# ilia-glushchenko/SimplePathTracer

Hardware: AMD Instinct MI355X
Metric: Msamples/s (pixels×spp/s), RTIOW random-sphere scene, 1/2/4/8 MI355X (higher is better)
Workload: dtype f32

## Files before the change

### simplepathtracer_amd/csrc/spt_batch.cpp

```cpp
#include "spt_host.h"

namespace spt_api {

int grow_host_rects(spt_ctx *ctx, BatchSet *bs, size_t n)
{
    if (bs->h_rects_cap >= n) return SPT_OK;
    if (int rc = svc_end(ctx)) return rc;
    const size_t cap = std::max<size_t>({n, 2 * bs->h_rects_cap, 64});
    if (bs->h_rects) HIP_TRY(ctx, hipHostFree(bs->h_rects));
    bs->h_rects = nullptr;
    bs->h_rects_cap = 0;
    HIP_TRY(ctx, hipHostMalloc((void **)&bs->h_rects, cap * sizeof(spt::BatchRect)));
    bs->h_rects_cap = cap;
    return SPT_OK;
}

void destroy_batch_set(BatchSet *b)
{
    if (b->d_rects) (void)hipFree(b->d_rects);
    if (b->h_rects) (void)hipHostFree(b->h_rects);
    if (b->d_stage) (void)hipFree(b->d_stage);
    if (b->stream) (void)hipStreamDestroy(b->stream);
}

// ... 154 lines not shown
    fa.spp_total = spp;
    fa.s_done = spp;
    fa.first = fa.last = 1;
    fa.mode = mode;
    fa.rects = bs->d_rects;
    fa.n_rects = (uint32_t)n;
    fa.inline_rects = inl ? 1u : 0u;
    if (inl)
        for (size_t i = 0; i < n; ++i) fa.rects_inline[i] = bs->h_rects[i];
    fa.head_reset = !use_svc ? w->d_head : nullptr;
    fa.head_queues = ra.n_queues;
    fa.prio = use_svc ? 0 : 1;
    EventPair ef = get_pair(ctx);
    HIP_TRY(ctx, hipEventRecord(ef.a, s));
    HIP_TRY(ctx, spt::launch_fold(fa, s));
    w->head_clean = !use_svc;
    HIP_TRY(ctx, hipEventRecord(ef.b, s));
    ctx->pending_fold.push_back(ef);

    for (size_t i = 0; i < n; ++i) {
        const BatchReq *r = batch[i];
        const spt::BatchRect &b = bs->h_rects[i];
        if (r->rgba)
            HIP_TRY(ctx, hipMemcpyAsync(r->rgba, bs->d_stage + b.pix_off, (size_t)b.npix * sizeof(float4),
                                        hipMemcpyDeviceToHost, s));
        if (r->g_data && !spec_d8 && b.rgb8 == ctx->d_frame8) {
            const size_t pitch = (size_t)W * 3, off = band_offset(W, H, r->yE, r->xB);
            HIP_TRY(ctx, hipMemcpy2DAsync(r->g_data + off, pitch, ctx->d_frame8 + off, pitch, (size_t)b.w * 3, b.rows,
                                          hipMemcpyDeviceToHost, s));
        }
    }
// ... 83 lines not shown
```

### simplepathtracer_amd/csrc/spt_ctx.cpp

```cpp
#include "spt_host.h"

namespace spt_api {

thread_local std::string g_thread_error;
thread_local const spt_ctx *t_in_callback = nullptr;

int fail(spt_ctx *ctx, int code, const char *fmt, ...)
{
    char buf[512];
    va_list ap;
    va_start(ap, fmt);
    vsnprintf(buf, sizeof buf, fmt, ap);
    va_end(ap);
    if (ctx) ctx->err = buf;
    g_thread_error = buf;
    return code;
}

void host_trace(const char *what, const void *arg)
{
    static const bool on = env_var("SPT_HOST_TRACE") && std::atoi(env_var("SPT_HOST_TRACE")) != 0;
    if (!on) return;
    static const auto t0 = std::chrono::steady_clock::now();
    const double ms = std::chrono::duration<double, std::milli>(std::chrono::steady_clock::now() - t0).count();
// ... 129 lines not shown
            uint32_t j = 0;
            while (x != 0.f && j < spt::kCodeSat) {
                x = x * 0.5f;
                ++j;
            }
            jz = std::max(jz, j);
        }
    return jz;
}

uint32_t code_jmax(const spt_ctx *ctx)
{
    return std::min(ctx->bounces > 0 ? ctx->bounces - 1u : 0u, ctx->code_jz);
}

spt::DeviceScene device_scene(const spt_ctx *ctx)
{
    return spt::DeviceScene{ctx->d_shade, ctx->d_mat, ctx->n, ctx->code_stride, code_jmax(ctx), ctx->accel};
}

int check_ready(spt_ctx *ctx)
{
    if (!ctx->scene_set) return fail(ctx, SPT_ERR_STATE, "scene not set (spt_set_scene)");
    if (!ctx->cam_set) return fail(ctx, SPT_ERR_STATE, "camera not set (spt_set_camera)");
    if (!ctx->params_set) return fail(ctx, SPT_ERR_STATE, "params not set (spt_set_params)");
    if (!spt::code_layout_fits(ctx->code_stride, code_jmax(ctx)))
        return fail(ctx, SPT_ERR_ARG,
                    "%u sphere slots at depth %u exceed the sample code space ((jmax + 1) * slots + 1 <= %u, jmax = %u)",
                    ctx->code_stride, ctx->bounces, spt::kCodeMax, code_jmax(ctx));
    return SPT_OK;
// ... 151 lines not shown
            shade[j] = ctx->h_shade[t.orig[j]];
            mat[j] = ctx->h_mat[t.orig[j]];
        }
    HIP_TRY(ctx, hipDeviceSynchronize());
    int rc = upload(ctx, &ctx->d_slots, &ctx->slots_cap, t.slots);
    if (!rc) rc = upload(ctx, &ctx->d_shade, &ctx->shade_cap, shade);
    if (!rc) rc = upload(ctx, &ctx->d_mat, &ctx->mat_cap, mat);
    if (!rc) rc = upload(ctx, &ctx->d_orig, &ctx->orig_cap, t.orig);
    if (!rc) rc = upload(ctx, &ctx->d_nodes, &ctx->nodes_cap, t.nodes);
    if (!rc) rc = upload(ctx, &ctx->d_kpre, &ctx->kpre_cap, t.kpre);
    if (rc) return rc;
    ctx->accel = spt::AccelView{ctx->d_slots, ctx->d_orig, ctx->d_nodes, t.always_groups, t.n_nodes,
                                t.n_nodes > t.leaves ? 1u : 0u, t.leaf_slots, ctx->d_kpre, t.pre_cm};
    ctx->code_stride = (uint32_t)std::max<size_t>(t.slots.size(), 1);
    ctx->code_jz = jz;
    ctx->tables = std::move(t);
    ctx->accel_gen++;
    ctx->accel_build_s = std::chrono::duration<double>(std::chrono::steady_clock::now() - t_start).count();
    return SPT_OK;
}

int wait_own_renders(spt_ctx *ctx)
{
    for (const EventPair &p : ctx->pending_render) HIP_TRY(ctx, hipEventSynchronize(p.b));
    return SPT_OK;
}

int rebuild_prim(spt_ctx *ctx)
{
    const bool want = ctx->prim_enabled && ctx->scene_set && ctx->cam_set && ctx->params_set &&
// ... 269 lines not shown
    if (const char *e = env_var("SPT_SVC_FULL_GRID"))
        if (std::atoi(e) != 0) {
            ctx->svc_grid = (uint32_t)(per_cu * ctx->num_cu);
            ctx->svc_full = true;
        }
    if (const char *e = env_var("SPT_BLOCKS_PER_CU")) per_cu = std::max(1, std::atoi(e));
    if (const char *e = env_var("SPT_CLAIM")) ctx->claim = (uint32_t)std::max(0, std::atoi(e));
    if (const char *e = env_var("SPT_CLUSTER_K")) ctx->cluster_k = (uint32_t)std::max(0, std::atoi(e));
    if (const char *e = env_var("SPT_TREE_B")) ctx->tree_branching = (uint32_t)std::max(0, std::atoi(e));
    if (const char *e = env_var("SPT_CLAIMS_PER_WAVE")) ctx->claims_per_wave = (uint32_t)std::max(1, std::atoi(e));
    if (const char *e = env_var("SPT_QUEUES"))
        ctx->queues = (uint32_t)std::min<int>((int)spt::kMaxQueues, std::max(1, std::atoi(e)));
    if (const char *e = env_var("SPT_WF_CAP")) ctx->wf_cap = (uint32_t)std::max(1024, std::atoi(e));
    if (const char *e = env_var("SPT_WF_QUEUE")) ctx->wf_queue = (uint32_t)std::min(8192, std::max(1, std::atoi(e) / 256)) * 256u;
    if (const char *e = env_var("SPT_HOST_GRID_DIV")) ctx->host_grid_div = (uint32_t)std::max(0, std::atoi(e));
    if (const char *e = env_var("SPT_BATCH")) ctx->batching = std::atoi(e) != 0;
    if (const char *e = env_var("SPT_READAHEAD")) ctx->readahead = std::atoi(e) != 0;
    if (const char *e = env_var("SPT_READAHEAD_PARTS"))
        ctx->spec.parts = (uint32_t)std::min(SpecFrame::kParts, std::max(1, std::atoi(e)));
    if (const char *e = env_var("SPT_BATCH_DBUF")) ctx->batch_dbuf = std::atoi(e) != 0;
    if (const char *e = env_var("SPT_BATCH_GRID_DIV")) ctx->batch_grid_div = (uint32_t)std::max(1, std::atoi(e));
    if (const char *e = env_var("SPT_BATCH_SETS"))
        ctx->batch_sets = (uint32_t)std::min<int>((int)kMaxBatchSets, std::max(1, std::atoi(e)));
    if (const char *e = env_var("SPT_HOST_SLOTS"))
        ctx->host_slots = (uint32_t)std::min<int>((int)kMaxHostSlots, std::max(1, std::atoi(e)));
    if (const char *e = env_var("SPT_SERVICE")) ctx->svc.enabled = std::atoi(e) != 0;
    if (const char *e = env_var("SPT_SVC_CLAIM")) ctx->svc.claim = (uint32_t)std::max(64, std::atoi(e) / 64 * 64);
    if (const char *e = env_var("SPT_SVC_LDS")) ctx->svc.lds = std::atoi(e) != 0;
    if (const char *e = env_var("SPT_SVC_QUEUES"))
        ctx->svc.queues = (uint32_t)std::min<int>((int)spt::kMaxQueues, std::max(1, std::atoi(e)));
// ... 315 lines not shown
```

### simplepathtracer_amd/csrc/spt_host.h

```cpp
#pragma once
#include "spt_hip.h"
#include "spt_accel.h"
#include "spt_internal.h"
#include "spt_readahead.h"

#include <hip/hip_runtime.h>

#include <algorithm>
#include <atomic>
#include <chrono>
#include <cmath>
#include <condition_variable>
#include <cstdarg>
#include <cstdint>
#include <cstdio>
#include <cstdlib>
#include <cstring>
#include <functional>
#include <mutex>
#include <string>
#include <thread>
#include <utility>
#include <vector>

// ... 166 lines not shown
    struct PrimKey {
        float view[12], eye[3];
        uint32_t W, H, prim_max;
        uint64_t accel_gen;
        bool valid;
        bool same(const PrimKey &o) const
        {
            return valid && o.valid && std::memcmp(view, o.view, sizeof view) == 0 &&
                   std::memcmp(eye, o.eye, sizeof eye) == 0 && W == o.W && H == o.H && prim_max == o.prim_max &&
                   accel_gen == o.accel_gen;
        }
    } prim_key{};
    uint64_t accel_gen = 0;
    uint32_t prim_blocks = 0, prim_entries = 0;
    uint32_t code_stride = 1, code_jz = 0;
    bool scene_set = false;
    std::vector<float> h_centers, h_radii;
    std::vector<float4> h_shade;
    std::vector<uint32_t> h_mat;
    uint32_t cluster_k = SPT_CLUSTER_AUTO;
    uint32_t tree_branching = SPT_TREE_AUTO;
    int engine = SPT_ENGINE_MEGAKERNEL;
    uint32_t wf_cap = 1u << 24;
    uint32_t wf_queue = 4096;
    spt::AccelView accel{};
    spt::Camera cam{};
    bool cam_set = false;
    uint32_t W = 0, H = 0, spp = 0, bounces = 0;
    uint64_t seed = 0;
    bool params_set = false;
// ... 92 lines not shown
int check_not_in_callback(spt_ctx *ctx);
int rebuild_prim(spt_ctx *ctx);
int wait_own_renders(spt_ctx *ctx);
int rebuild_accel(spt_ctx *ctx);
int ensure_wavefront(spt_ctx *ctx, Workspace *w, uint32_t cap, uint32_t qcap);
hipStream_t companion_for(spt_ctx *ctx, hipStream_t s);
Workspace * workspace_for(spt_ctx *ctx, hipStream_t s);
uint32_t render_grid(const spt_ctx *ctx, uint64_t items, uint32_t claim, uint32_t div, bool masked = false);
uint32_t claim_size(const spt_ctx *ctx, uint64_t items, bool masked = false);
int masked_for(spt_ctx *ctx, hipStream_t s, spt_ctx::Masked **out);
uint32_t full_grid(const spt_ctx *ctx, bool masked = false);
uint64_t fmix64(uint64_t z);
int check_ready(spt_ctx *ctx);
spt::DeviceScene device_scene(const spt_ctx *ctx);
uint32_t code_jmax(const spt_ctx *ctx);
uint32_t halvings_to_zero(const std::vector<float4> &shade);
double busy_ms(const spt_ctx *ctx);
int collect_timings(spt_ctx *ctx, bool wait = true);
EventPair get_pair(spt_ctx *ctx);
int check_on_device(spt_ctx *ctx, const void *p, const char *what);
int fail(spt_ctx *ctx, int code, const char *fmt, ...);
int svc_retire(spt_ctx *ctx, hipStream_t s, uint64_t w0, uint64_t words, uint32_t idx);
int svc_submit(spt_ctx *ctx, const spt::RenderArgs &ra, int mode, hipStream_t s, uint64_t *w0_out, uint32_t *idx_out);
int svc_submit_jobs(spt_ctx *ctx, int mode, const SvcJobSpec *jobs, size_t n, uint64_t total_slots, hipStream_t s, uint64_t *w0_out, uint32_t *idx_out);
bool svc_eligible(const spt_ctx *ctx, uint64_t words, bool keep_samples);
void host_trace(const char *what, const void *arg = nullptr);
void warm_start(spt_ctx *ctx);
hipStream_t warm_take(spt_ctx *ctx, int i);
void warm_join(spt_ctx *ctx);
uint32_t svc_session_grid(const spt_ctx *ctx);
// ... 68 lines not shown
```

### simplepathtracer_amd/csrc/spt_internal.h

```cpp
#pragma once
#include <hip/hip_runtime.h>
#include <stdint.h>

#include "spt_hip.h"

namespace spt {

struct RowMap {
    uint32_t y0, y1, strip, parts, part;
    uint32_t x0, width;
};

__host__ __device__ inline uint32_t row_of(const RowMap &m, uint32_t lr)
{
    uint32_t blk = lr / m.strip;
    return m.y0 + (blk * m.parts + m.part) * m.strip + (lr - blk * m.strip);
}

__host__ __device__ inline uint32_t rows_owned(const RowMap &m)
{
    if (m.y1 <= m.y0) return 0;
    uint32_t h = m.y1 - m.y0;
    uint32_t period = m.strip * m.parts;
    uint32_t full = h / period, rem = h % period;
// ... 25 lines not shown
        const uint32_t t = qb / th;
        if (t < ft) {
            const uint32_t e = qb - t * th;
            row = e >> 3;
            c = (t << 3) | (e & 7u);
        } else {
            const uint32_t e = qb - ft * th;
            row = e / wr;
            c = (ft << 3) + (e - row * wr);
        }
    }
    lr = (band << 3) + row;
    col = c;
}

struct FastDiv {
    uint32_t d, m, s;
};
inline FastDiv make_fastdiv(uint32_t d)
{
    FastDiv f{d, 0u, 0u};
    if (d <= 1u) return f;
    uint32_t l = 0;
    while ((1ull << l) < d) ++l;
    f.m = (uint32_t)(((1ull << (31 + l)) / d) + 1ull);
    f.s = l - 1u;
    return f;
}
__host__ __device__ inline uint32_t fast_div(uint32_t x, const FastDiv &f)
{
#ifdef __HIP_DEVICE_COMPILE__
    const uint32_t hi = __umulhi(x, f.m);
#else
    const uint32_t hi = (uint32_t)(((uint64_t)x * f.m) >> 32);
#endif
    return f.d <= 1u ? x : hi >> f.s;
}

__host__ __device__ inline uint32_t row_of_fast(const RowMap &m, uint32_t lr, const FastDiv &div_strip)
{
    const uint32_t blk = fast_div(lr, div_strip);
    return m.y0 + (blk * m.parts + m.part) * m.strip + (lr - blk * m.strip);
}

__host__ __device__ inline void ts_item(uint32_t q, uint32_t width, uint32_t rows, uint32_t S, const FastDiv &div_band,
                                        const FastDiv &div_tile, uint32_t &sl, uint32_t &lr, uint32_t &col)
{
    const uint32_t band = rows >= 8u ? fast_div(q, div_band) : 0u;
    const uint32_t h = rows - (band << 3) < 8u ? rows - (band << 3) : 8u;
    const uint32_t qb = q - band * 8u * width * S;
    const uint32_t ft = width >> 3, wr = width & 7u;
    const uint32_t ti = h * 8u * S;
    uint32_t e, wt, c0;
// ... 24 lines not shown
}

__host__ __device__ inline void ts_slot_base(uint32_t lr, uint32_t col, uint32_t width, uint32_t rows, uint32_t S,
                                             uint32_t &q0, uint32_t &step)
{
    const uint32_t band = lr >> 3;
    const uint32_t h = rows - (band << 3) < 8u ? rows - (band << 3) : 8u;
    const uint32_t ft = width >> 3, wr = width & 7u;
    const uint32_t t = col >> 3;
    const uint32_t tc = t < ft ? t : ft;
    const uint32_t wt = t < ft ? 8u : wr;
    q0 = band * 8u * width * S + tc * h * 8u * S + (lr - (band << 3)) * wt + (col - (tc << 3));
    step = h * wt;
}

constexpr uint32_t kCodeSmall = 0x33800000u;
constexpr uint32_t kCodeMax = 2u * (kCodeSmall - 1u);
constexpr uint32_t kCodeSat = 280;
__host__ __device__ inline bool code_layout_fits(uint64_t stride, uint32_t jmax)
{
    return (jmax + 1ull) * stride + 1ull <= kCodeMax;
}
__host__ __device__ inline uint32_t diffuse_code(uint32_t j, uint32_t slot, uint32_t stride)
{
    return 2u + j * stride + slot;
}
__host__ __device__ inline void diffuse_decode(uint32_t c, const FastDiv &div, uint32_t &j, uint32_t &slot)
{
    const uint32_t v = c - 2u;
    j = fast_div(v, div);
    slot = v - j * div.d;
}
__host__ __device__ inline uint32_t code_word(uint32_t c)
{
    return c < kCodeSmall ? c : 0x80000000u | (c - kCodeSmall + 1u);
}
__host__ __device__ inline uint32_t word_code(uint32_t w)
{
    const uint32_t a = w & 0x7FFFFFFFu;
    if (a == 0u || a >= kCodeSmall) return 0u;
    return (w >> 31) ? a + kCodeSmall - 1u : a;
}
constexpr uint32_t kZeroWord = 1u;

constexpr uint32_t kMaxGroup = 16;
constexpr uint32_t kClusterSlots = 8;
constexpr uint32_t kFlatLeafSlots = 4;
constexpr double kFlatScale = 1.0 - 1e-4;
constexpr double kBoxS = 1.63e-3;
constexpr float kBoxMinDir = 0x1p-20f;
constexpr uint32_t kNoSlot = 0xFFFFFFFFu;
constexpr uint32_t kMiss = 0xFFFFFFFFu;

struct AccelView {
    const float4 *slots;
    const uint32_t *orig;
    const void *nodes;
    uint32_t always_groups, n_nodes;
// ... 94 lines not shown
constexpr uint32_t kSvcHostCommitted = 0, kSvcHostClosing = 32, kSvcHostPub = 64, kSvcHostStop = 96,
                   kSvcHostWatchdog = 128, kSvcHostWords = 160;
constexpr uint32_t kSvcTraceClaims = 1u << 21;
hipError_t launch_render_svc(const RenderArgs &a, uint32_t grid, hipStream_t s);
bool svc_supported(const AccelView &ac);
bool svc_lds(const AccelView &ac);
uint32_t svc_lds_grid(bool full);
uint32_t svc_block(const AccelView &ac);

struct FoldArgs {
    const uint32_t *samples;
    uint32_t slot_words;
    const float4 *shade;
    float sky[3];
    FastDiv code_div;
    float4 *acc;
    float4 *out_rgba;
    uint8_t *out_rgb8;
    RowMap map;
    uint32_t width, height, npix, spp_batch, spp_total;
    uint32_t s_done;
    int first, last, mode;
    int preview;
    int prio;
    int alias;
    const BatchRect *rects;
    uint32_t n_rects;
    uint32_t range_alias, out_i0, alias_h, src_rows;
    uint32_t *head_reset;
    uint32_t head_queues;
// ... 40 lines not shown
```

### simplepathtracer_amd/csrc/spt_kernels.hip

```cpp
#include "spt_path.h"

#include <algorithm>
#include <mutex>

namespace spt {


#ifndef SPT_WAVES_PER_EU
#define SPT_WAVES_PER_EU 0
#endif
#ifndef SPT_NUM_SGPR
#define SPT_NUM_SGPR 96
#endif
#if SPT_WAVES_PER_EU
#define SPT_RENDER_ATTR __attribute__((amdgpu_waves_per_eu(SPT_WAVES_PER_EU, SPT_WAVES_PER_EU)))
#elif SPT_NUM_SGPR
#define SPT_CAP_WAVES (800 / (((SPT_NUM_SGPR - 2 + 15) / 16) * 16 + 16) > 8 ? 8 : 800 / (((SPT_NUM_SGPR - 2 + 15) / 16) * 16 + 16))
#define SPT_RENDER_ATTR __attribute__((amdgpu_num_sgpr(SPT_NUM_SGPR), amdgpu_waves_per_eu(SPT_CAP_WAVES)))
#else
#define SPT_RENDER_ATTR
#endif

#ifndef SPT_LDS_BLOCK
#define SPT_LDS_BLOCK 1024
// ... 160 lines not shown
        const uint32_t j = cur + lane;
        const uint32_t v = j < njobs ? __hip_atomic_load(jc + j, __ATOMIC_RELAXED, __HIP_MEMORY_SCOPE_AGENT) : 0xFFFFFFFFu;
        const unsigned long long le = __ballot(v <= nb);
        if (le != ~0ull || cur + 64u >= njobs) {
            if (le != 0ull) cur += 63u - (uint32_t)__builtin_clzll(le);
            break;
        }
        cur += 64u;
    }
    const gu32 *src = (const gu32 *)(k.svc_jobs + cur);
    const uint32_t w = lane < 24u ? __hip_atomic_load(src + lane, __ATOMIC_RELAXED, __HIP_MEMORY_SCOPE_AGENT) : 0u;
    if (lane < 24u) rec[lane] = w;
    return __builtin_amdgcn_readfirstlane(cur);
}

__device__ __forceinline__ float halve_n(float x, uint32_t j)
{
    if (j <= 126u) {
        const float r = x * __uint_as_float((127u - j) << 23);
        if (__builtin_fabsf(r) >= 0x1p-126f || x == 0.f || !__builtin_isfinite(x)) return r;
    }
    for (uint32_t i = 0; i < j; ++i) x = x * 0.5f;
    return x;
}
__device__ __forceinline__ f3 decode_sample(const FoldArgs &a, uint32_t w)
{
    const uint32_t c = word_code(w);
    if (c == 0u) {
        const float k = __uint_as_float(w);
        return mul(mk(a.sky[0] * k, a.sky[1] * k, a.sky[2] * k), 0.5f);
    }
    if (c == 1u) return mk(0.f, 0.f, 0.f);
    uint32_t j, slot;
    diffuse_decode(c, a.code_div, j, slot);
    const float4 sh = a.shade[slot];
    return mk(halve_n(sh.x * 0.5f, j), halve_n(sh.y * 0.5f, j), halve_n(sh.z * 0.5f, j));
}

template <int N>
__device__ __forceinline__ void decode_run(const FoldArgs &a, const uint32_t (&w)[N], f3 (&col)[N])
{
    uint32_t c[N], j[N];
    float4 sh[N];
#pragma unroll
    for (int i = 0; i < N; ++i) {
        c[i] = word_code(w[i]);
        uint32_t slot;
        diffuse_decode(c[i] >= 2u ? c[i] : 2u, a.code_div, j[i], slot);
        sh[i] = a.shade[slot];
    }
#pragma unroll
    for (int i = 0; i < N; ++i) {
        const float k = __uint_as_float(w[i]);
        const f3 s = mul(mk(a.sky[0] * k, a.sky[1] * k, a.sky[2] * k), 0.5f);
        const f3 d = mk(halve_n(sh[i].x * 0.5f, j[i]), halve_n(sh[i].y * 0.5f, j[i]), halve_n(sh[i].z * 0.5f, j[i]));
        col[i] = c[i] == 0u ? s : c[i] == 1u ? mk(0.f, 0.f, 0.f) : d;
    }
}

#ifndef SPT_FOLD_RUN
#define SPT_FOLD_RUN 8
#endif
constexpr int kFoldDecode = SPT_FOLD_RUN < 8 ? SPT_FOLD_RUN : 8;
static_assert(SPT_FOLD_RUN % kFoldDecode == 0, "fold runs are decoded kFoldDecode words at a time");

__device__ __forceinline__ void alias_accumulate(const FoldArgs &a, const uint32_t *samples, uint32_t p, uint32_t W,
                                                 uint32_t H, uint32_t row0, uint32_t rows, uint32_t S, float4 &acc)
{
    const uint32_t dy_lo = p >= W ? (p - W + H) / H : 0u;
    const uint32_t dy_hi = min(H - 1u, p / H);
    const uint32_t ns = dy_hi + 1u - dy_lo;
    const uint2 *s2 = (const uint2 *)samples;
    auto add = [&](uint32_t w) {
        const f3 c = decode_sample(a, w);
        acc.x = acc.x + c.x;
        acc.y = acc.y + c.y;
        acc.z = acc.z + c.z;
        acc.w = acc.w + 1.f;
    };
    constexpr uint32_t kSrc = 4;
    if (ns <= kSrc) {
        uint32_t sq[kSrc], sst[kSrc];
#pragma unroll
        for (uint32_t j = 0; j < kSrc; ++j) {
            const uint32_t dy = j < ns ? dy_lo + j : dy_lo;
            ts_slot_base(dy - row0, p - dy * H, W, rows, S, sq[j], sst[j]);
        }
        const bool rev = W < H;
        for (uint32_t k = 0; k < S; ++k) {
// ... 32 lines not shown
                    const uint32_t key = s2[q].y;
                    const uint64_t kp = ((uint64_t)key << 32) | (dy * W + dx);
                    if (key != 0u && kp > prev && kp < best) {
                        best = kp;
                        best_slot = q;
                    }
                }
                if (best == ~0ull) break;
                add(s2[best_slot].x);
                prev = best;
            }
        }
    }
}

__device__ __forceinline__ void fold_pixel(const FoldArgs &a, const uint32_t *samples, const RowMap &map,
                                           uint32_t rows, int alias, uint32_t lr, uint32_t col, float4 *out_rgba,
                                           uint8_t *out_rgb8)
{
    const uint32_t W = map.width, S = a.spp_batch;
    const uint32_t p = lr * W + col;
    float4 acc = a.first ? make_float4(0.f, 0.f, 0.f, 0.f) : a.acc[p];
    uint32_t q0, step;
    ts_slot_base(lr, col, W, rows, S, q0, step);
    if (a.mode == 0) {
        constexpr int kFoldRun = SPT_FOLD_RUN;
        uint32_t k = 0;
        for (; k + kFoldRun <= S; k += kFoldRun) {
            uint32_t w[kFoldRun];
#pragma unroll
            for (int i = 0; i < kFoldRun; ++i) w[i] = samples[q0 + (k + i) * step];
#pragma unroll
            for (int g = 0; g < kFoldRun; g += kFoldDecode) {
                uint32_t w8[kFoldDecode];
#pragma unroll
                for (int i = 0; i < kFoldDecode; ++i) w8[i] = w[g + i];
                f3 c[kFoldDecode];
                decode_run<kFoldDecode>(a, w8, c);
#pragma unroll
                for (int i = 0; i < kFoldDecode; ++i) {
                    acc.x = acc.x + c[i].x;
                    acc.y = acc.y + c[i].y;
                    acc.z = acc.z + c[i].z;
                    acc.w = acc.w + 1.f;
                }
            }
        }
        for (; k < S; ++k) {
            const f3 c = decode_sample(a, samples[q0 + k * step]);
            acc.x = acc.x + c.x;
            acc.y = acc.y + c.y;
            acc.z = acc.z + c.z;
            acc.w = acc.w + 1.f;
        }
    } else if (!alias) {
        const uint2 *s2 = (const uint2 *)samples;
        for (uint32_t k = 0; k < S; ++k) {
            const uint2 v = s2[q0 + k * step];
            if (v.y != 0u) {
                const f3 c = decode_sample(a, v.x);
                acc.x = acc.x + c.x;
                acc.y = acc.y + c.y;
                acc.z = acc.z + c.z;
                acc.w = acc.w + 1.f;
            }
        }
    } else {
        alias_accumulate(a, samples, p, W, rows, 0u, rows, S, acc);
    }
    if (!a.last) {
        a.acc[p] = acc;
        if (!a.preview) return;
    }
    const float scale = a.mode == 0 ? 1.f / (float)a.s_done : 1.f / acc.w;
    const float r = acc.x * scale, g = acc.y * scale, b = acc.z * scale;
    if (out_rgba) out_rgba[p] = make_float4(r, g, b, 0.f);
    if (out_rgb8) {
        const uint32_t x = map.x0 + col;
        const uint32_t y = row_of(map, lr);
        const size_t gi = (size_t)3 * ((size_t)(a.height - 1u - y) * a.width + x);
        out_rgb8[gi + 0] = gamma_byte(r);
        out_rgb8[gi + 1] = gamma_byte(g);
        out_rgb8[gi + 2] = gamma_byte(b);
// ... 502 lines not shown
{
    render_body<true, (int)kClusterSlots, true, kLdsBlock>(a);
}
__global__ __launch_bounds__(kLdsBlock)
    __attribute__((amdgpu_num_sgpr(SPT_LDS_NUM_SGPR), amdgpu_waves_per_eu(2 * kLdsBlock / 256))) void render_kernel_lds_batch(RenderArgs a)
{
    render_body<true, (int)kClusterSlots, true, kLdsBlock, true>(a);
}

__global__ __launch_bounds__(kLdsBlock)
    __attribute__((amdgpu_num_sgpr(SPT_LDS_NUM_SGPR), amdgpu_waves_per_eu(2 * kLdsBlock / 256))) void render_kernel_svc_lds(RenderArgs a)
{
    render_body<true, (int)kClusterSlots, true, kLdsBlock, false, false, true>(a);
}

#ifndef SPT_FOLD_PRIO
#define SPT_FOLD_PRIO 3
#endif
#ifndef SPT_FOLD_BLOCK
#define SPT_FOLD_BLOCK 256
#endif
__global__ __launch_bounds__(SPT_FOLD_BLOCK) void fold_kernel(FoldArgs a)
{
    if (a.prio) __builtin_amdgcn_s_setprio(SPT_FOLD_PRIO);
    const uint32_t i = blockIdx.x * blockDim.x + threadIdx.x;
    if (i >= a.npix) return;
    const uint32_t rows = a.npix / a.map.width;
    uint32_t lr, col;
    tile_pixel(i, a.map.width, rows, lr, col);
    fold_pixel(a, a.samples, a.map, rows, a.alias, lr, col, a.out_rgba, a.out_rgb8);
}

__global__ __launch_bounds__(256) void fold_alias_range_kernel(FoldArgs a)
{
    if (a.prio) __builtin_amdgcn_s_setprio(3);
    const uint32_t t = blockIdx.x * blockDim.x + threadIdx.x;
    if (t >= a.npix) return;
    float4 acc = a.first ? make_float4(0.f, 0.f, 0.f, 0.f) : a.acc[t];
    alias_accumulate(a, a.samples, a.out_i0 + t, a.map.width, a.alias_h, a.map.y0, a.src_rows, a.spp_batch, acc);
    if (!a.last) {
        a.acc[t] = acc;
        if (!a.preview) return;
    }
    const float scale = 1.f / acc.w;
    if (a.out_rgba) a.out_rgba[t] = make_float4(acc.x * scale, acc.y * scale, acc.z * scale, 0.f);
}

typedef __attribute__((address_space(4))) const BatchRect crect_k;
__device__ __forceinline__ uint32_t fold_rect(crect_k *rs, uint32_t n, uint32_t i)
{
    uint32_t lo = 0, hi = n;
    while (hi - lo > 1u) {
        const uint32_t mid = (lo + hi) >> 1;
        if (rs[mid].pix_off <= i) lo = mid; else hi = mid;
    }
    return lo;
}

__global__ __launch_bounds__(256) void fold_kernel_batch(FoldArgs a)
{
#ifndef SPT_FOLD_PRIO_BATCH
#define SPT_FOLD_PRIO_BATCH 1
#endif
    if (SPT_FOLD_PRIO_BATCH && a.prio) __builtin_amdgcn_s_setprio(3);
    const uint32_t i = blockIdx.x * blockDim.x + threadIdx.x;
    if (blockIdx.x == 0 && a.head_reset && threadIdx.x < a.head_queues) a.head_reset[threadIdx.x * kQueueStride] = 0u;
    if (i >= a.npix) return;
    typedef __attribute__((address_space(4))) const FoldArgs cfold_t;
    typedef __attribute__((address_space(4))) const char kchar;
    cfold_t *ka = (cfold_t *)(kchar *)__builtin_amdgcn_kernarg_segment_ptr();
    crect_k *rs = a.inline_rects ? (crect_k *)ka->rects_inline : (crect_k *)a.rects;
    crect_k &r = rs[fold_rect(rs, a.n_rects, i)];
    const RowMap map{r.y0, r.y0 + r.rows, 1u, 1u, 0u, r.x0, r.w};
    uint32_t lr, col;
    tile_pixel(i - r.pix_off, r.w, r.rows, lr, col);
    fold_pixel(a, a.samples + (size_t)a.slot_words * r.slot_off, map, r.rows, (int)r.alias, lr, col,
               a.out_rgba ? a.out_rgba + r.pix_off : nullptr, r.rgb8);
}

__global__ __launch_bounds__(256) void expand_kernel(FoldArgs a, float4 *out, uint32_t p0, uint32_t n)
{
    const uint32_t i = blockIdx.x * blockDim.x + threadIdx.x;
    if (i >= n) return;
    const uint32_t p = p0 + i;
    const uint32_t W = a.map.width, rows = a.npix / W, lr = p / W, col = p - lr * W;
    uint32_t q0, step;
    ts_slot_base(lr, col, W, rows, a.spp_batch, q0, step);
    for (uint32_t k = 0; k < a.spp_batch; ++k) {
        const uint32_t q = q0 + k * step;
        const uint32_t w = a.slot_words == 1u ? a.samples[q] : a.samples[2u * q];
        const bool counted = a.slot_words == 1u || a.samples[2u * q + 1u] != 0u;
        const f3 c = decode_sample(a, w);
        out[(size_t)i * a.spp_batch + k] = make_float4(c.x, c.y, c.z, counted ? 1.f : 0.f);
    }
}

__global__ __launch_bounds__(256) void assemble_kernel(const float4 *tiles, uint32_t max_rows, RowMap base,
                                                       uint32_t width, uint32_t height, float4 *frame, uint8_t *rgb8)
{
    const uint32_t x = blockIdx.x * blockDim.x + threadIdx.x;
    const uint32_t k = blockIdx.y;
    const uint32_t r = blockIdx.z;
    if (x >= base.width) return;
    RowMap m = base;
    m.part = r;
    if (k >= rows_owned(m)) return;
    const uint32_t y = row_of(m, k);
// ... 129 lines not shown
        return hipGetLastError();
    }
    if (a.scene.accel.tree)
        hipLaunchKernelGGL((render_kernel_svc<true, (int)kClusterSlots>), dim3(grid), dim3(kRenderBlock), 0, s, a);
    else if (a.scene.accel.leaf_slots == kFlatLeafSlots)
        hipLaunchKernelGGL((render_kernel_svc<false, (int)kFlatLeafSlots>), dim3(grid), dim3(kRenderBlock), 0, s, a);
    else
        hipLaunchKernelGGL((render_kernel_svc<false, (int)kClusterSlots>), dim3(grid), dim3(kRenderBlock), 0, s, a);
    return hipGetLastError();
}


hipError_t launch_fold(const FoldArgs &a, hipStream_t s)
{
    if (a.npix == 0) return hipSuccess;
    if (a.range_alias)
        hipLaunchKernelGGL(fold_alias_range_kernel, dim3((a.npix + 255) / 256), dim3(256), 0, s, a);
    else if (a.rects)
        hipLaunchKernelGGL(fold_kernel_batch, dim3((a.npix + 255) / 256), dim3(256), 0, s, a);
    else
        hipLaunchKernelGGL(fold_kernel, dim3((a.npix + SPT_FOLD_BLOCK - 1) / SPT_FOLD_BLOCK), dim3(SPT_FOLD_BLOCK), 0, s, a);
    return hipGetLastError();
}

hipError_t launch_expand(const FoldArgs &a, float4 *out, uint32_t p0, uint32_t n, hipStream_t s)
{
    if (n == 0) return hipSuccess;
    hipLaunchKernelGGL(expand_kernel, dim3((n + 255) / 256), dim3(256), 0, s, a, out, p0, n);
    return hipGetLastError();
}

hipError_t launch_assemble(const float4 *tiles, uint32_t max_rows, RowMap base, uint32_t width, uint32_t height,
                           float4 *frame, uint8_t *rgb8, hipStream_t s)
{
    if (max_rows == 0 || base.width == 0) return hipSuccess;
    dim3 grid((base.width + 255) / 256, max_rows, base.parts);
    hipLaunchKernelGGL(assemble_kernel, grid, dim3(256), 0, s, tiles, max_rows, base, width, height, frame, rgb8);
    return hipGetLastError();
}

hipError_t launch_selftest(const float *a, const float *b, const uint32_t *bits, uint32_t n, float *out, hipStream_t s)
{
    if (n == 0) return hipSuccess;
// ... 31 lines not shown
```

### simplepathtracer_amd/csrc/spt_render.cpp

```cpp
#include "spt_host.h"

namespace spt_api {

spt::FoldArgs fold_args(const spt_ctx *ctx, const uint32_t *samples, uint32_t slot_words)
{
    spt::FoldArgs fa{};
    fa.samples = samples;
    fa.slot_words = slot_words;
    fa.shade = ctx->d_shade;
    for (int j = 0; j < 3; ++j) fa.sky[j] = ctx->cam.sky[j];
    fa.code_div = spt::make_fastdiv(ctx->code_stride);
    return fa;
}

int render_impl(spt_ctx *ctx, int mode, const spt::RowMap &map, float4 *d_rgba, uint8_t *d_rgb8, hipStream_t s,
                bool keep_samples, const Progress *pg, uint32_t grid_div, const AliasRange *ar)
{
    const uint32_t rows = spt::rows_owned(map);
    const uint64_t npix64 = (uint64_t)rows * map.width;
    if (npix64 == 0 && ar && ar->n) {
        spt::FoldArgs fa = fold_args(ctx, nullptr, 2u);
        fa.out_rgba = d_rgba;
        fa.map = map;
        fa.width = ctx->W;
        fa.height = ctx->H;
        fa.npix = ar->n;
// ... 101 lines not shown
            ra.head = w->d_head;
        }
        ra.spp_batch = b;
        ra.s0 = s0;
        ra.n_items = npix * b;
        ra.n_queues = ctx->queues;
        {
            const uint32_t per = (ra.n_items + ra.n_queues - 1u) / ra.n_queues;
            ra.queue_items = (per + ra.claim - 1u) / ra.claim * ra.claim;
        }
        ra.div_band = spt::make_fastdiv(rows >= 8 ? 8u * map.width * b : 1u);
        ra.div_tile = spt::make_fastdiv(64u * b);
        EventPair ev = get_pair(ctx);
        uint64_t svc_w0 = 0;
        uint32_t svc_idx = 0;
        if (use_svc) {
            if (!ctx->ref_recorded) {
                HIP_TRY(ctx, hipEventRecord(ctx->ref_ev, s));
                ctx->ref_recorded = true;
            }
            HIP_TRY(ctx, hipEventRecord(ev.a, s));
            if ((rc = svc_submit(ctx, ra, mode, s, &svc_w0, &svc_idx))) return rc;
            HIP_TRY(ctx, hipEventRecord(ev.b, s));
            fa.samples = ctx->svc.d_ring + svc_w0;
        } else if (ctx->engine == SPT_ENGINE_WAVEFRONT) {
            const uint64_t blocks = spt::wavefront_blocks(ctx->accel, ctx->device);
            if (blocks == 0) return fail(ctx, SPT_ERR_HIP, "wavefront engine: no resident blocks");
            const uint32_t cap = (uint32_t)std::min<uint64_t>(std::min<uint64_t>(ctx->wf_cap, blocks * ctx->wf_queue),
                                                               std::max<uint32_t>(ra.n_items, 1024u));
            if ((rc = ensure_wavefront(ctx, w, cap, ctx->wf_queue))) return rc;
            HIP_TRY(ctx, hipEventRecord(ev.a, s));
            if (!ctx->ref_recorded) {
                HIP_TRY(ctx, hipEventRecord(ctx->ref_ev, s));
                ctx->ref_recorded = true;
            }
            HIP_TRY(ctx, spt::launch_wavefront(w->wf, ra, s));
            HIP_TRY(ctx, hipEventRecord(ev.b, s));
        } else {
            HIP_TRY(ctx, hipMemsetAsync(w->d_head, 0, sizeof(uint32_t) * spt::kQueueStride * ra.n_queues, s));
            if (!ctx->ref_recorded) {
                HIP_TRY(ctx, hipEventRecord(ctx->ref_ev, s));
                ctx->ref_recorded = true;
            }
            HIP_TRY(ctx, hipEventRecord(ev.a, s));
            spt::LaunchShape sh{render_grid(ctx, ra.n_items, ra.claim, grid_div, mk_ != nullptr), ctx->block, grid_div, 0, 0};
            HIP_TRY(ctx, spt::launch_render(ra, sh, s));
            ctx->last_grid = sh.ran_grid;
            ctx->last_block = sh.ran_block;
            HIP_TRY(ctx, hipEventRecord(ev.b, s));
        }
        ctx->pending_render.push_back(ev);
        ctx->launches++;
        if (keep_samples) continue;
        fa.spp_batch = b;
        fa.first = s0 == 0;
        fa.last = s0 + b >= ctx->spp;
        fa.s_done = s0 + b;
        EventPair ef = get_pair(ctx);
        if (s2 && j > 0) HIP_TRY(ctx, hipStreamWaitEvent(s, ctx->dbuf_fold, 0));
        fa.prio = use_svc ? 0 : 1;
        HIP_TRY(ctx, hipEventRecord(ef.a, s));
        HIP_TRY(ctx, spt::launch_fold(fa, s));
        HIP_TRY(ctx, hipEventRecord(ef.b, s));
        if (s2) HIP_TRY(ctx, hipEventRecord(ctx->dbuf_fold, s));
        ctx->pending_fold.push_back(ef);
        if (use_svc && (rc = svc_retire(ctx, s, svc_w0, (uint64_t)npix * b * slot_words, svc_idx))) return rc;
        if (pg && pg->after_pass) {
            const int r = pg->after_pass(s0 + b);
            if (r < 0) return r;
            if (r > 0) break;
        }
    }
    if (s2 && s != s_caller) HIP_TRY(ctx, hipStreamWaitEvent(s_caller, ctx->dbuf_fold, 0));
    if (mk_) {
        HIP_TRY(ctx, hipEventRecord(mk_->done, mk_->stream));
        HIP_TRY(ctx, hipStreamWaitEvent(s_caller, mk_->done, 0));
    }
// ... 260 lines not shown
```

Measured before the change: 23150.

## Add fast fold decode path, software-pipeline sample loads, skip per-pass head memset

On the host, compute a bound on how many halvings of the scene's shade colours stay normal floats. When the maximum bounce depth fits within that bound, the fold kernels run a templated FAST path that decodes diffuse samples with a single exponent multiply and branch-free selects, with no denormal fallback loop. The fold loop now loads the next group of four sample words while the current group is decoded, with scheduling barriers around it. The render path also drops the hipMemsetAsync of the queue heads when the previous fold kernel already reset them, which removes one extra stream operation per pass but adds state tracking of head_clean across batch and render paths.

```diff
diff --git a/simplepathtracer_amd/csrc/spt_batch.cpp b/simplepathtracer_amd/csrc/spt_batch.cpp
--- a/simplepathtracer_amd/csrc/spt_batch.cpp
+++ b/simplepathtracer_amd/csrc/spt_batch.cpp
@@ -192,7 +192,7 @@
     EventPair ef = get_pair(ctx);
     HIP_TRY(ctx, hipEventRecord(ef.a, s));
     HIP_TRY(ctx, spt::launch_fold(fa, s));
-    w->head_clean = !use_svc;
+    if (!use_svc && fa.npix) w->head_clean = true;
     HIP_TRY(ctx, hipEventRecord(ef.b, s));
     ctx->pending_fold.push_back(ef);
 
diff --git a/simplepathtracer_amd/csrc/spt_codes.h b/simplepathtracer_amd/csrc/spt_codes.h
--- /dev/null
+++ b/simplepathtracer_amd/csrc/spt_codes.h
@@ -0,0 +1,113 @@
+#pragma once
+#include <stddef.h>
+#include <stdint.h>
+
+#if defined(__HIPCC__)
+#define SPT_HD __host__ __device__
+#else
+#define SPT_HD
+#endif
+
+namespace spt {
+
+struct FastDiv {
+    uint32_t d, m, s;
+};
+inline FastDiv make_fastdiv(uint32_t d)
+{
+    FastDiv f{d, 0u, 0u};
+    if (d <= 1u) return f;
+    uint32_t l = 0;
+    while ((1ull << l) < d) ++l;
+    f.m = (uint32_t)(((1ull << (31 + l)) / d) + 1ull);
+    f.s = l - 1u;
+    return f;
+}
+SPT_HD inline uint32_t fast_div(uint32_t x, const FastDiv &f)
+{
+#ifdef __HIP_DEVICE_COMPILE__
+    const uint32_t hi = __umulhi(x, f.m);
+#else
+    const uint32_t hi = (uint32_t)(((uint64_t)x * f.m) >> 32);
+#endif
+    return f.d <= 1u ? x : hi >> f.s;
+}
+
+constexpr uint32_t kCodeSmall = 0x33800000u;
+constexpr uint32_t kCodeMax = 2u * (kCodeSmall - 1u);
+constexpr uint32_t kCodeSat = 280;
+SPT_HD inline bool code_layout_fits(uint64_t stride, uint32_t jmax)
+{
+    return (jmax + 1ull) * stride + 1ull <= kCodeMax;
+}
+SPT_HD inline uint32_t diffuse_code(uint32_t j, uint32_t slot, uint32_t stride)
+{
+    return 2u + j * stride + slot;
+}
+SPT_HD inline void diffuse_decode(uint32_t c, const FastDiv &div, uint32_t &j, uint32_t &slot)
+{
+    const uint32_t v = c - 2u;
+    j = fast_div(v, div);
+    slot = v - j * div.d;
+}
+SPT_HD inline uint32_t code_word(uint32_t c)
+{
+    return c < kCodeSmall ? c : 0x80000000u | (c - kCodeSmall + 1u);
+}
+SPT_HD inline uint32_t word_code(uint32_t w)
+{
+    const uint32_t a = w & 0x7FFFFFFFu;
+    if (a == 0u || a >= kCodeSmall) return 0u;
+    return (w >> 31) ? a + kCodeSmall - 1u : a;
+}
+constexpr uint32_t kZeroWord = 1u;
+
+SPT_HD inline float bits_float(uint32_t u)
+{
+    float f;
+    __builtin_memcpy(&f, &u, sizeof f);
+    return f;
+}
+SPT_HD inline uint32_t float_bits(float f)
+{
+    uint32_t u;
+    __builtin_memcpy(&u, &f, sizeof u);
+    return u;
+}
+
+constexpr uint32_t kFastHalvings = 126;
+SPT_HD inline float halve_n(float x, uint32_t j)
+{
+    if (j <= kFastHalvings) {
+        const float r = x * bits_float((127u - j) << 23);
+        if (__builtin_fabsf(r) >= 0x1p-126f || x == 0.f || !__builtin_isfinite(x)) return r;
+    }
+    for (uint32_t i = 0; i < j; ++i) x = x * 0.5f;
+    return x;
+}
+SPT_HD inline float halve_fast(float x, uint32_t j)
+{
+    return x * bits_float((127u - j) << 23);
+}
+
+SPT_HD inline uint32_t fast_halvings(float h)
+{
+    const uint32_t a = float_bits(h) & 0x7FFFFFFFu, e = a >> 23;
+    if (a == 0u || e == 255u) return kFastHalvings;
+    if (e == 0u) return 0u;
+    return e - 1u < kFastHalvings ? e - 1u : kFastHalvings;
+}
+
+inline uint32_t fast_decode_bound(const float *shade4, size_t n, uint32_t jmax)
+{
+    uint32_t jf = jmax < kFastHalvings ? jmax : kFastHalvings;
+    for (size_t i = 0; i < n; ++i)
+        for (int c = 0; c < 3; ++c) {
+            volatile float h = shade4[4 * i + c] * 0.5f;
+            const uint32_t f = fast_halvings(h);
+            jf = f < jf ? f : jf;
+        }
+    return jf;
+}
+
+}
diff --git a/simplepathtracer_amd/csrc/spt_ctx.cpp b/simplepathtracer_amd/csrc/spt_ctx.cpp
--- a/simplepathtracer_amd/csrc/spt_ctx.cpp
+++ b/simplepathtracer_amd/csrc/spt_ctx.cpp
@@ -167,6 +167,11 @@
     return std::min(ctx->bounces > 0 ? ctx->bounces - 1u : 0u, ctx->code_jz);
 }
 
+uint32_t code_jfast(const spt_ctx *ctx)
+{
+    return std::min(code_jmax(ctx), ctx->code_jf);
+}
+
 spt::DeviceScene device_scene(const spt_ctx *ctx)
 {
     return spt::DeviceScene{ctx->d_shade, ctx->d_mat, ctx->n, ctx->code_stride, code_jmax(ctx), ctx->accel};
@@ -348,6 +353,8 @@
                                 t.n_nodes > t.leaves ? 1u : 0u, t.leaf_slots, ctx->d_kpre, t.pre_cm};
     ctx->code_stride = (uint32_t)std::max<size_t>(t.slots.size(), 1);
     ctx->code_jz = jz;
+    ctx->code_jf = spt::fast_decode_bound(ctx->h_shade.empty() ? nullptr : &ctx->h_shade[0].x, ctx->h_shade.size(),
+                                          spt::kFastHalvings);
     ctx->tables = std::move(t);
     ctx->accel_gen++;
     ctx->accel_build_s = std::chrono::duration<double>(std::chrono::steady_clock::now() - t_start).count();
@@ -647,6 +654,7 @@
     if (const char *e = env_var("SPT_WF_CAP")) ctx->wf_cap = (uint32_t)std::max(1024, std::atoi(e));
     if (const char *e = env_var("SPT_WF_QUEUE")) ctx->wf_queue = (uint32_t)std::min(8192, std::max(1, std::atoi(e) / 256)) * 256u;
     if (const char *e = env_var("SPT_HOST_GRID_DIV")) ctx->host_grid_div = (uint32_t)std::max(0, std::atoi(e));
+    if (const char *e = env_var("SPT_FOLD_SLOW")) ctx->fold_slow = std::atoi(e) != 0;
     if (const char *e = env_var("SPT_BATCH")) ctx->batching = std::atoi(e) != 0;
     if (const char *e = env_var("SPT_READAHEAD")) ctx->readahead = std::atoi(e) != 0;
     if (const char *e = env_var("SPT_READAHEAD_PARTS"))
diff --git a/simplepathtracer_amd/csrc/spt_host.h b/simplepathtracer_amd/csrc/spt_host.h
--- a/simplepathtracer_amd/csrc/spt_host.h
+++ b/simplepathtracer_amd/csrc/spt_host.h
@@ -204,6 +204,8 @@
     uint64_t accel_gen = 0;
     uint32_t prim_blocks = 0, prim_entries = 0;
     uint32_t code_stride = 1, code_jz = 0;
+    uint32_t code_jf = 0;
+    bool fold_slow = false;
     bool scene_set = false;
     std::vector<float> h_centers, h_radii;
     std::vector<float4> h_shade;
@@ -326,6 +328,7 @@
 int check_ready(spt_ctx *ctx);
 spt::DeviceScene device_scene(const spt_ctx *ctx);
 uint32_t code_jmax(const spt_ctx *ctx);
+uint32_t code_jfast(const spt_ctx *ctx);
 uint32_t halvings_to_zero(const std::vector<float4> &shade);
 double busy_ms(const spt_ctx *ctx);
 int collect_timings(spt_ctx *ctx, bool wait = true);
diff --git a/simplepathtracer_amd/csrc/spt_internal.h b/simplepathtracer_amd/csrc/spt_internal.h
--- a/simplepathtracer_amd/csrc/spt_internal.h
+++ b/simplepathtracer_amd/csrc/spt_internal.h
@@ -2,6 +2,7 @@
 #include <hip/hip_runtime.h>
 #include <stdint.h>
 
+#include "spt_codes.h"
 #include "spt_hip.h"
 
 namespace spt {
@@ -63,29 +64,6 @@
     col = c;
 }
 
-struct FastDiv {
-    uint32_t d, m, s;
-};
-inline FastDiv make_fastdiv(uint32_t d)
-{
-    FastDiv f{d, 0u, 0u};
-    if (d <= 1u) return f;
-    uint32_t l = 0;
-    while ((1ull << l) < d) ++l;
-    f.m = (uint32_t)(((1ull << (31 + l)) / d) + 1ull);
-    f.s = l - 1u;
-    return f;
-}
-__host__ __device__ inline uint32_t fast_div(uint32_t x, const FastDiv &f)
-{
-#ifdef __HIP_DEVICE_COMPILE__
-    const uint32_t hi = __umulhi(x, f.m);
-#else
-    const uint32_t hi = (uint32_t)(((uint64_t)x * f.m) >> 32);
-#endif
-    return f.d <= 1u ? x : hi >> f.s;
-}
-
 __host__ __device__ inline uint32_t row_of_fast(const RowMap &m, uint32_t lr, const FastDiv &div_strip)
 {
     const uint32_t blk = fast_div(lr, div_strip);
@@ -140,34 +118,6 @@
     step = h * wt;
 }
 
-constexpr uint32_t kCodeSmall = 0x33800000u;
-constexpr uint32_t kCodeMax = 2u * (kCodeSmall - 1u);
-constexpr uint32_t kCodeSat = 280;
-__host__ __device__ inline bool code_layout_fits(uint64_t stride, uint32_t jmax)
-{
-    return (jmax + 1ull) * stride + 1ull <= kCodeMax;
-}
-__host__ __device__ inline uint32_t diffuse_code(uint32_t j, uint32_t slot, uint32_t stride)
-{
-    return 2u + j * stride + slot;
-}
-__host__ __device__ inline void diffuse_decode(uint32_t c, const FastDiv &div, uint32_t &j, uint32_t &slot)
-{
-    const uint32_t v = c - 2u;
-    j = fast_div(v, div);
-    slot = v - j * div.d;
-}
-__host__ __device__ inline uint32_t code_word(uint32_t c)
-{
-    return c < kCodeSmall ? c : 0x80000000u | (c - kCodeSmall + 1u);
-}
-__host__ __device__ inline uint32_t word_code(uint32_t w)
-{
-    const uint32_t a = w & 0x7FFFFFFFu;
-    if (a == 0u || a >= kCodeSmall) return 0u;
-    return (w >> 31) ? a + kCodeSmall - 1u : a;
-}
-constexpr uint32_t kZeroWord = 1u;
 
 constexpr uint32_t kMaxGroup = 16;
 constexpr uint32_t kClusterSlots = 8;
@@ -292,6 +242,8 @@
     const float4 *shade;
     float sky[3];
     FastDiv code_div;
+    uint32_t jfast;
+    int fast;
     float4 *acc;
     float4 *out_rgba;
     uint8_t *out_rgb8;
diff --git a/simplepathtracer_amd/csrc/spt_kernels.hip b/simplepathtracer_amd/csrc/spt_kernels.hip
--- a/simplepathtracer_amd/csrc/spt_kernels.hip
+++ b/simplepathtracer_amd/csrc/spt_kernels.hip
@@ -198,15 +198,16 @@
     return __builtin_amdgcn_readfirstlane(cur);
 }
 
-__device__ __forceinline__ float halve_n(float x, uint32_t j)
-{
-    if (j <= 126u) {
-        const float r = x * __uint_as_float((127u - j) << 23);
-        if (__builtin_fabsf(r) >= 0x1p-126f || x == 0.f || !__builtin_isfinite(x)) return r;
-    }
-    for (uint32_t i = 0; i < j; ++i) x = x * 0.5f;
-    return x;
-}
+template <bool FAST>
+__device__ __forceinline__ f3 diffuse_colour(const float4 &sh, uint32_t j)
+{
+    if (FAST) {
+        const float k = bits_float((127u - j) << 23);
+        return mk(sh.x * 0.5f * k, sh.y * 0.5f * k, sh.z * 0.5f * k);
+    }
+    return mk(halve_n(sh.x * 0.5f, j), halve_n(sh.y * 0.5f, j), halve_n(sh.z * 0.5f, j));
+}
+template <bool FAST>
 __device__ __forceinline__ f3 decode_sample(const FoldArgs &a, uint32_t w)
 {
     const uint32_t c = word_code(w);
@@ -217,15 +218,13 @@
     if (c == 1u) return mk(0.f, 0.f, 0.f);
     uint32_t j, slot;
     diffuse_decode(c, a.code_div, j, slot);
-    const float4 sh = a.shade[slot];
-    return mk(halve_n(sh.x * 0.5f, j), halve_n(sh.y * 0.5f, j), halve_n(sh.z * 0.5f, j));
+    return diffuse_colour<FAST>(a.shade[slot], j);
 }
 
 template <int N>
-__device__ __forceinline__ void decode_run(const FoldArgs &a, const uint32_t (&w)[N], f3 (&col)[N])
-{
-    uint32_t c[N], j[N];
-    float4 sh[N];
+__device__ __forceinline__ void decode_gather(const FoldArgs &a, const uint32_t (&w)[N], uint32_t (&c)[N],
+                                              uint32_t (&j)[N], float4 (&sh)[N])
+{
 #pragma unroll
     for (int i = 0; i < N; ++i) {
         c[i] = word_code(w[i]);
@@ -233,21 +232,40 @@
         diffuse_decode(c[i] >= 2u ? c[i] : 2u, a.code_div, j[i], slot);
         sh[i] = a.shade[slot];
     }
+}
+template <bool FAST, int N>
+__device__ __forceinline__ void decode_add(const FoldArgs &a, const uint32_t (&w)[N], const uint32_t (&c)[N],
+                                           const uint32_t (&j)[N], const float4 (&sh)[N], float4 &acc)
+{
 #pragma unroll
     for (int i = 0; i < N; ++i) {
         const float k = __uint_as_float(w[i]);
+        const bool sky = c[i] == 0u, zero = c[i] == 1u;
+        if (FAST) {
+            const float m1 = __builtin_unpredictable(sky) ? k : 0.5f;
+            const float m2 = __builtin_unpredictable(sky) ? 0.5f : bits_float((127u - j[i]) << 23);
+            const float x = (__builtin_unpredictable(sky) ? a.sky[0] : sh[i].x) * m1 * m2;
+            const float y = (__builtin_unpredictable(sky) ? a.sky[1] : sh[i].y) * m1 * m2;
+            const float z = (__builtin_unpredictable(sky) ? a.sky[2] : sh[i].z) * m1 * m2;
+            acc.x = acc.x + (__builtin_unpredictable(zero) ? 0.f : x);
+            acc.y = acc.y + (__builtin_unpredictable(zero) ? 0.f : y);
+            acc.z = acc.z + (__builtin_unpredictable(zero) ? 0.f : z);
+            acc.w = acc.w + 1.f;
+            continue;
+        }
         const f3 s = mul(mk(a.sky[0] * k, a.sky[1] * k, a.sky[2] * k), 0.5f);
-        const f3 d = mk(halve_n(sh[i].x * 0.5f, j[i]), halve_n(sh[i].y * 0.5f, j[i]), halve_n(sh[i].z * 0.5f, j[i]));
-        col[i] = c[i] == 0u ? s : c[i] == 1u ? mk(0.f, 0.f, 0.f) : d;
-    }
-}
-
-#ifndef SPT_FOLD_RUN
-#define SPT_FOLD_RUN 8
-#endif
-constexpr int kFoldDecode = SPT_FOLD_RUN < 8 ? SPT_FOLD_RUN : 8;
-static_assert(SPT_FOLD_RUN % kFoldDecode == 0, "fold runs are decoded kFoldDecode words at a time");
-
+        const f3 d = diffuse_colour<FAST>(sh[i], j[i]);
+        acc.x = acc.x + (__builtin_unpredictable(sky) ? s.x : __builtin_unpredictable(zero) ? 0.f : d.x);
+        acc.y = acc.y + (__builtin_unpredictable(sky) ? s.y : __builtin_unpredictable(zero) ? 0.f : d.y);
+        acc.z = acc.z + (__builtin_unpredictable(sky) ? s.z : __builtin_unpredictable(zero) ? 0.f : d.z);
+        acc.w = acc.w + 1.f;
+    }
+}
+
+constexpr int kFoldDecode = 4;
+constexpr int kFoldAhead = 1;
+
+template <bool FAST>
 __device__ __forceinline__ void alias_accumulate(const FoldArgs &a, const uint32_t *samples, uint32_t p, uint32_t W,
                                                  uint32_t H, uint32_t row0, uint32_t rows, uint32_t S, float4 &acc)
 {
@@ -256,7 +274,7 @@
     const uint32_t ns = dy_hi + 1u - dy_lo;
     const uint2 *s2 = (const uint2 *)samples;
     auto add = [&](uint32_t w) {
-        const f3 c = decode_sample(a, w);
+        const f3 c = decode_sample<FAST>(a, w);
         acc.x = acc.x + c.x;
         acc.y = acc.y + c.y;
         acc.z = acc.z + c.z;
@@ -319,6 +337,7 @@
     }
 }
 
+template <bool FAST>
 __device__ __forceinline__ void fold_pixel(const FoldArgs &a, const uint32_t *samples, const RowMap &map,
                                            uint32_t rows, int alias, uint32_t lr, uint32_t col, float4 *out_rgba,
                                            uint8_t *out_rgb8)
@@ -329,30 +348,25 @@
     uint32_t q0, step;
     ts_slot_base(lr, col, W, rows, S, q0, step);
     if (a.mode == 0) {
-        constexpr int kFoldRun = SPT_FOLD_RUN;
-        uint32_t k = 0;
-        for (; k + kFoldRun <= S; k += kFoldRun) {
-            uint32_t w[kFoldRun];
+        static_assert(kFoldAhead == 1, "one run of words is loaded ahead");
+        const uint32_t runs = S / kFoldDecode;
+        uint32_t w[kFoldDecode];
 #pragma unroll
-            for (int i = 0; i < kFoldRun; ++i) w[i] = samples[q0 + (k + i) * step];
+        for (int i = 0; i < kFoldDecode; ++i) w[i] = runs ? samples[q0 + (uint32_t)i * step] : 0u;
+        for (uint32_t r = 0; r < runs; ++r) {
+            uint32_t cur[kFoldDecode], c[kFoldDecode], j[kFoldDecode];
+            float4 sh[kFoldDecode];
 #pragma unroll
-            for (int g = 0; g < kFoldRun; g += kFoldDecode) {
-                uint32_t w8[kFoldDecode];
+            for (int i = 0; i < kFoldDecode; ++i) cur[i] = w[i];
+            decode_gather<kFoldDecode>(a, cur, c, j, sh);
+            __builtin_amdgcn_sched_barrier(0);
 #pragma unroll
-                for (int i = 0; i < kFoldDecode; ++i) w8[i] = w[g + i];
-                f3 c[kFoldDecode];
-                decode_run<kFoldDecode>(a, w8, c);
-#pragma unroll
-                for (int i = 0; i < kFoldDecode; ++i) {
-                    acc.x = acc.x + c[i].x;
-                    acc.y = acc.y + c[i].y;
-                    acc.z = acc.z + c[i].z;
-                    acc.w = acc.w + 1.f;
-                }
-            }
-        }
-        for (; k < S; ++k) {
-            const f3 c = decode_sample(a, samples[q0 + k * step]);
+            for (int i = 0; i < kFoldDecode; ++i) w[i] = samples[q0 + min((r + 1u) * kFoldDecode + i, S - 1u) * step];
+            __builtin_amdgcn_sched_barrier(0);
+            decode_add<FAST, kFoldDecode>(a, cur, c, j, sh, acc);
+        }
+        for (uint32_t k = runs * kFoldDecode; k < S; ++k) {
+            const f3 c = decode_sample<FAST>(a, samples[q0 + k * step]);
             acc.x = acc.x + c.x;
             acc.y = acc.y + c.y;
             acc.z = acc.z + c.z;
@@ -363,7 +377,7 @@
         for (uint32_t k = 0; k < S; ++k) {
             const uint2 v = s2[q0 + k * step];
             if (v.y != 0u) {
-                const f3 c = decode_sample(a, v.x);
+                const f3 c = decode_sample<FAST>(a, v.x);
                 acc.x = acc.x + c.x;
                 acc.y = acc.y + c.y;
                 acc.z = acc.z + c.z;
@@ -371,7 +385,7 @@
             }
         }
     } else {
-        alias_accumulate(a, samples, p, W, rows, 0u, rows, S, acc);
+        alias_accumulate<FAST>(a, samples, p, W, rows, 0u, rows, S, acc);
     }
     if (!a.last) {
         a.acc[p] = acc;
@@ -904,30 +918,32 @@
     render_body<true, (int)kClusterSlots, true, kLdsBlock, false, false, true>(a);
 }
 
-#ifndef SPT_FOLD_PRIO
-#define SPT_FOLD_PRIO 3
-#endif
-#ifndef SPT_FOLD_BLOCK
-#define SPT_FOLD_BLOCK 256
-#endif
-__global__ __launch_bounds__(SPT_FOLD_BLOCK) void fold_kernel(FoldArgs a)
-{
-    if (a.prio) __builtin_amdgcn_s_setprio(SPT_FOLD_PRIO);
+__device__ __forceinline__ void fold_prologue(const FoldArgs &a)
+{
+    if (a.prio) __builtin_amdgcn_s_setprio(3);
+    if (blockIdx.x == 0 && a.head_reset && threadIdx.x < a.head_queues) a.head_reset[threadIdx.x * kQueueStride] = 0u;
+}
+
+template <bool FAST>
+__global__ __launch_bounds__(256) __attribute__((amdgpu_waves_per_eu(8))) void fold_kernel(FoldArgs a)
+{
+    fold_prologue(a);
     const uint32_t i = blockIdx.x * blockDim.x + threadIdx.x;
     if (i >= a.npix) return;
     const uint32_t rows = a.npix / a.map.width;
     uint32_t lr, col;
     tile_pixel(i, a.map.width, rows, lr, col);
-    fold_pixel(a, a.samples, a.map, rows, a.alias, lr, col, a.out_rgba, a.out_rgb8);
-}
-
+    fold_pixel<FAST>(a, a.samples, a.map, rows, a.alias, lr, col, a.out_rgba, a.out_rgb8);
+}
+
+template <bool FAST>
 __global__ __launch_bounds__(256) void fold_alias_range_kernel(FoldArgs a)
 {
-    if (a.prio) __builtin_amdgcn_s_setprio(3);
+    fold_prologue(a);
     const uint32_t t = blockIdx.x * blockDim.x + threadIdx.x;
     if (t >= a.npix) return;
     float4 acc = a.first ? make_float4(0.f, 0.f, 0.f, 0.f) : a.acc[t];
-    alias_accumulate(a, a.samples, a.out_i0 + t, a.map.width, a.alias_h, a.map.y0, a.src_rows, a.spp_batch, acc);
+    alias_accumulate<FAST>(a, a.samples, a.out_i0 + t, a.map.width, a.alias_h, a.map.y0, a.src_rows, a.spp_batch, acc);
     if (!a.last) {
         a.acc[t] = acc;
         if (!a.preview) return;
@@ -947,14 +963,11 @@
     return lo;
 }
 
+template <bool FAST>
 __global__ __launch_bounds__(256) void fold_kernel_batch(FoldArgs a)
 {
-#ifndef SPT_FOLD_PRIO_BATCH
-#define SPT_FOLD_PRIO_BATCH 1
-#endif
-    if (SPT_FOLD_PRIO_BATCH && a.prio) __builtin_amdgcn_s_setprio(3);
+    fold_prologue(a);
     const uint32_t i = blockIdx.x * blockDim.x + threadIdx.x;
-    if (blockIdx.x == 0 && a.head_reset && threadIdx.x < a.head_queues) a.head_reset[threadIdx.x * kQueueStride] = 0u;
     if (i >= a.npix) return;
     typedef __attribute__((address_space(4))) const FoldArgs cfold_t;
     typedef __attribute__((address_space(4))) const char kchar;
@@ -964,10 +977,11 @@
     const RowMap map{r.y0, r.y0 + r.rows, 1u, 1u, 0u, r.x0, r.w};
     uint32_t lr, col;
     tile_pixel(i - r.pix_off, r.w, r.rows, lr, col);
-    fold_pixel(a, a.samples + (size_t)a.slot_words * r.slot_off, map, r.rows, (int)r.alias, lr, col,
+    fold_pixel<FAST>(a, a.samples + (size_t)a.slot_words * r.slot_off, map, r.rows, (int)r.alias, lr, col,
                a.out_rgba ? a.out_rgba + r.pix_off : nullptr, r.rgb8);
 }
 
+template <bool FAST>
 __global__ __launch_bounds__(256) void expand_kernel(FoldArgs a, float4 *out, uint32_t p0, uint32_t n)
 {
     const uint32_t i = blockIdx.x * blockDim.x + threadIdx.x;
@@ -980,7 +994,7 @@
         const uint32_t q = q0 + k * step;
         const uint32_t w = a.slot_words == 1u ? a.samples[q] : a.samples[2u * q];
         const bool counted = a.slot_words == 1u || a.samples[2u * q + 1u] != 0u;
-        const f3 c = decode_sample(a, w);
+        const f3 c = decode_sample<FAST>(a, w);
         out[(size_t)i * a.spp_batch + k] = make_float4(c.x, c.y, c.z, counted ? 1.f : 0.f);
     }
 }
@@ -1140,19 +1154,25 @@
 hipError_t launch_fold(const FoldArgs &a, hipStream_t s)
 {
     if (a.npix == 0) return hipSuccess;
-    if (a.range_alias)
-        hipLaunchKernelGGL(fold_alias_range_kernel, dim3((a.npix + 255) / 256), dim3(256), 0, s, a);
-    else if (a.rects)
-        hipLaunchKernelGGL(fold_kernel_batch, dim3((a.npix + 255) / 256), dim3(256), 0, s, a);
-    else
-        hipLaunchKernelGGL(fold_kernel, dim3((a.npix + SPT_FOLD_BLOCK - 1) / SPT_FOLD_BLOCK), dim3(SPT_FOLD_BLOCK), 0, s, a);
+    const dim3 grid((a.npix + 255) / 256), block(256);
+    if (a.range_alias) {
+        if (a.fast) hipLaunchKernelGGL(fold_alias_range_kernel<true>, grid, block, 0, s, a);
+        else hipLaunchKernelGGL(fold_alias_range_kernel<false>, grid, block, 0, s, a);
+    } else if (a.rects) {
+        if (a.fast) hipLaunchKernelGGL(fold_kernel_batch<true>, grid, block, 0, s, a);
+        else hipLaunchKernelGGL(fold_kernel_batch<false>, grid, block, 0, s, a);
+    } else {
+        if (a.fast) hipLaunchKernelGGL(fold_kernel<true>, grid, block, 0, s, a);
+        else hipLaunchKernelGGL(fold_kernel<false>, grid, block, 0, s, a);
+    }
     return hipGetLastError();
 }
 
 hipError_t launch_expand(const FoldArgs &a, float4 *out, uint32_t p0, uint32_t n, hipStream_t s)
 {
     if (n == 0) return hipSuccess;
-    hipLaunchKernelGGL(expand_kernel, dim3((n + 255) / 256), dim3(256), 0, s, a, out, p0, n);
+    if (a.fast) hipLaunchKernelGGL(expand_kernel<true>, dim3((n + 255) / 256), dim3(256), 0, s, a, out, p0, n);
+    else hipLaunchKernelGGL(expand_kernel<false>, dim3((n + 255) / 256), dim3(256), 0, s, a, out, p0, n);
     return hipGetLastError();
 }
 
diff --git a/simplepathtracer_amd/csrc/spt_render.cpp b/simplepathtracer_amd/csrc/spt_render.cpp
--- a/simplepathtracer_amd/csrc/spt_render.cpp
+++ b/simplepathtracer_amd/csrc/spt_render.cpp
@@ -10,6 +10,8 @@
     fa.shade = ctx->d_shade;
     for (int j = 0; j < 3; ++j) fa.sky[j] = ctx->cam.sky[j];
     fa.code_div = spt::make_fastdiv(ctx->code_stride);
+    fa.jfast = code_jfast(ctx);
+    fa.fast = fa.jfast >= code_jmax(ctx) && !ctx->fold_slow;
     return fa;
 }
 
@@ -141,6 +143,7 @@
         EventPair ev = get_pair(ctx);
         uint64_t svc_w0 = 0;
         uint32_t svc_idx = 0;
+        bool launched = false;
         if (use_svc) {
             if (!ctx->ref_recorded) {
                 HIP_TRY(ctx, hipEventRecord(ctx->ref_ev, s));
@@ -164,7 +167,10 @@
             HIP_TRY(ctx, spt::launch_wavefront(w->wf, ra, s));
             HIP_TRY(ctx, hipEventRecord(ev.b, s));
         } else {
-            HIP_TRY(ctx, hipMemsetAsync(w->d_head, 0, sizeof(uint32_t) * spt::kQueueStride * ra.n_queues, s));
+            if (!w->head_clean)
+                HIP_TRY(ctx, hipMemsetAsync(w->d_head, 0, sizeof(uint32_t) * spt::kQueueStride * ra.n_queues, s));
+            w->head_clean = false;
+            launched = true;
             if (!ctx->ref_recorded) {
                 HIP_TRY(ctx, hipEventRecord(ctx->ref_ev, s));
                 ctx->ref_recorded = true;
@@ -186,8 +192,11 @@
         EventPair ef = get_pair(ctx);
         if (s2 && j > 0) HIP_TRY(ctx, hipStreamWaitEvent(s, ctx->dbuf_fold, 0));
         fa.prio = use_svc ? 0 : 1;
+        fa.head_reset = launched ? w->d_head : nullptr;
+        fa.head_queues = ra.n_queues;
         HIP_TRY(ctx, hipEventRecord(ef.a, s));
         HIP_TRY(ctx, spt::launch_fold(fa, s));
+        if (launched && fa.npix) w->head_clean = true;
         HIP_TRY(ctx, hipEventRecord(ef.b, s));
         if (s2) HIP_TRY(ctx, hipEventRecord(ctx->dbuf_fold, s));
         ctx->pending_fold.push_back(ef);
```

After: 23370 (median of 6 runs). No clear change (+0.9%).
